# Codeuser0717/CVAE-GAN

Measured on NVIDIA B200. Metric: train_samples_per_s, higher is better.
Workload: dtype f32

## Files before the change

cvae_gan_b200/csrc/chain.cuh:

```cuda
#pragma once
#include "gemm.cuh"
#include "misc_kernels.cuh"

namespace cvg {

constexpr int CH_TM = 32;
constexpr int CH_THREADS = 256;
constexpr int CH_NB = 64;
constexpr int CH_KC = 64;
constexpr int CH_H0 = 256, CH_H1 = 128, CH_H2 = 64;
constexpr int CH_MAX_IN = 256;
constexpr int CH_MAX_K = 32;
constexpr int CH_WBUF = 2 * CH_KC * CH_NB;

struct CriticChainArgs {
  int M = 0, ld = 0, F = 0;
  const float* x = nullptr;
  long long sx = 0;
  const float* W[4] = {};
  int ldw[4] = {};
  const float* b[4] = {};
  const float* wlabel = nullptr;
  int ldwl = 0;
  const float* inv_sigma = nullptr;
  const uint8_t* m1 = nullptr;
  const uint8_t* m2 = nullptr;
  float keep_inv = 1.f, slope = 0.2f;
  float* a[3] = {};
  float* s = nullptr;
  float* g[3] = {};
  double* osum = nullptr;
  float seed[2] = {0.f, 0.f};
};

struct ClassifierChainArgs {
  int M = 0, ld = 0, F = 0, K = 0, label = 0;
  const float* x = nullptr;
  long long sx = 0;
  const float* W[4] = {};
  const float* b[4] = {};
  const float* gamma = nullptr;
  const float* beta = nullptr;
  float ln_eps = 1e-5f;
  const uint8_t* m1 = nullptr;
  const uint8_t* m2 = nullptr;
  float keep_inv = 1.f;
  float *a1 = nullptr, *h2 = nullptr, *a2 = nullptr, *rs = nullptr, *a3 = nullptr, *logit = nullptr, *dlogit = nullptr;
  float* g[3] = {};
  float coef = 1.f;
  double* loss = nullptr;
  float* dgamma = nullptr;
  float* dbeta = nullptr;
  unsigned long long* acc = nullptr;
  unsigned* cnt = nullptr;
};

template <bool WT, class Ep>
__device__ __forceinline__ void chain_layer(const float* X, const float* __restrict__ W, int ldw, int R, int N, float* wbuf,
                                            Ep ep) {
  const int tid = threadIdx.x;
  const int grp = tid >> 6, t64 = tid & 63;
  const int tm = (t64 & 7) * 4, tn = (t64 >> 3) * 8;
  const int Rp = (R + TBK - 1) / TBK * TBK;
  const int nkc = (Rp + CH_KC - 1) / CH_KC;
  const bool wvec = (ldw & 3) == 0;
  for (int n0 = 0; n0 < N; n0 += CH_NB) {
    float4 pre[4];
    auto gload = [&](int kc) {
#pragma unroll
      for (int j = 0; j < 4; ++j) pre[j] = make_float4(0.f, 0.f, 0.f, 0.f);
      if (WT) {
        const int n = n0 + (tid & 63);
        if (n >= N) return;
#pragma unroll
        for (int j = 0; j < 4; ++j) {
          const int k = kc + (tid >> 6) * 16 + 4 * j;
          const float* src = W + (size_t)n * ldw + k;
          if (wvec && k + 3 < R) {
            pre[j] = ld4(src);
          } else {
            if (k < R) pre[j].x = src[0];
            if (k + 1 < R) pre[j].y = src[1];
            if (k + 2 < R) pre[j].z = src[2];
            if (k + 3 < R) pre[j].w = src[3];
          }
        }
      } else {
// ... 114 lines not shown
    return tot;
  }
};

struct DactEp {
  float scale;
  const uint8_t* mask;
  float keep_inv;
  float neg;
  const float* A;
  float* Y;
  float* S;
  int ld, m0, M;
  __device__ __forceinline__ void operator()(int n, int m, float4 v) const {
    float y[4] = {v.x, v.y, v.z, v.w};
    const size_t off = (size_t)n * ld + m0 + m;
    float keep[4] = {1.f, 1.f, 1.f, 1.f};
    if (mask) {
      const uchar4 mk = *reinterpret_cast<const uchar4*>(mask + off);
      keep[0] = ep_keep(mk.x, keep_inv);
      keep[1] = ep_keep(mk.y, keep_inv);
      keep[2] = ep_keep(mk.z, keep_inv);
      keep[3] = ep_keep(mk.w, keep_inv);
    }
#pragma unroll
    for (int i = 0; i < 4; ++i) y[i] = ep_dact(y[i], scale, keep[i], A[n * CH_TM + m + i], neg);
    st4(Y + off, make_float4(y[0], y[1], y[2], y[3]));
    if (S)
#pragma unroll
      for (int i = 0; i < 4; ++i) S[n * CH_TM + m + i] = m0 + m + i < M ? y[i] : 0.f;
  }
};

__device__ __forceinline__ void chain_stage(float* S, int rows, const float* src, int nvalid, int ld, int m0, int M) {
  for (int i = threadIdx.x; i < rows * CH_TM; i += CH_THREADS) {
    const int k = i / CH_TM, m = i % CH_TM;
    S[i] = (k < nvalid && m0 + m < M) ? src[(size_t)k * ld + m0 + m] : 0.f;
  }
}

__host__ __device__ inline int chain_x_rows(int F, int K) {
  const int fp = (F + TBK - 1) / TBK * TBK;
  const int kp = 2 * ((K + TBK - 1) / TBK * TBK);
  return fp > kp ? fp : kp;
}
inline size_t critic_chain_smem(int F) {
  return sizeof(float) * ((size_t)CH_WBUF + (size_t)(CH_H0 + CH_H1 + CH_H2) * CH_TM + (size_t)chain_x_rows(F, 1) * CH_TM);
}
inline size_t classifier_chain_smem(int F, int K) {
  return sizeof(float) * ((size_t)CH_WBUF + (size_t)(CH_H0 + 2 * CH_H1 + CH_H2) * CH_TM + (size_t)chain_x_rows(F, K) * CH_TM);
}

__global__ void __launch_bounds__(CH_THREADS, 2) critic_chain_kernel(const CriticChainArgs g) {
  extern __shared__ __align__(16) float ch_smem[];
  float* wbuf = ch_smem;
  float* A0 = wbuf + CH_WBUF;
  float* A1 = A0 + CH_H0 * CH_TM;
  float* A2 = A1 + CH_H1 * CH_TM;
  float* X = A2 + CH_H2 * CH_TM;
  const int pass = blockIdx.y, m0 = blockIdx.x * CH_TM;
  const int M = g.M, ld = g.ld;
  const size_t ps0 = (size_t)pass * CH_H0 * ld, ps1 = (size_t)pass * CH_H1 * ld, ps2 = (size_t)pass * CH_H2 * ld;

  chain_stage(X, (g.F + TBK - 1) / TBK * TBK, g.x + (long long)pass * g.sx, g.F, ld, m0, M);
  __syncthreads();
  chain_layer<true>(X, g.W[0], g.ldw[0], g.F, CH_H0, wbuf,
                    FwdEp{g.b[0], g.wlabel, g.ldwl, g.inv_sigma[0 + pass], ACT_LRELU, g.slope, g.m1 + ps0, g.keep_inv,
                          g.a[0] + ps0, A0, ld, m0, M});
  chain_layer<true>(A0, g.W[1], g.ldw[1], CH_H0, CH_H1, wbuf,
                    FwdEp{g.b[1], nullptr, 0, g.inv_sigma[2 + pass], ACT_LRELU, g.slope, g.m2 + ps1, g.keep_inv,
                          g.a[1] + ps1, A1, ld, m0, M});
  chain_layer<true>(A1, g.W[2], g.ldw[2], CH_H1, CH_H2, wbuf,
                    FwdEp{g.b[2], nullptr, 0, g.inv_sigma[4 + pass], ACT_LRELU, g.slope, nullptr, 1.f,
                          g.a[2] + ps2, A2, ld, m0, M});
  double tot = 0.0;
  const FwdEp score{g.b[3], nullptr, 0, g.inv_sigma[6 + pass], ACT_NONE, g.slope, nullptr, 1.f,
                    g.s + (size_t)pass * ld, nullptr, ld, m0, M};
  chain_layer<true>(A2, g.W[3], g.ldw[3], CH_H2, 1, wbuf, [&](int n, int m, float4 y) { tot += score(n, m, y); });
  tot = warp_sum_d(tot);
  if (threadIdx.x == 0) atomicAdd(g.osum + pass, tot);
  for (int i = threadIdx.x; i < TBK * CH_TM; i += CH_THREADS)
    X[i] = (i < CH_TM && m0 + i < M) ? g.seed[pass] : 0.f;
  __syncthreads();
  chain_layer<false>(X, g.W[3], g.ldw[3], 1, CH_H2, wbuf,
                     DactEp{g.inv_sigma[6 + pass], nullptr, 1.f, g.slope, A2, g.g[2] + ps2, A2, ld, m0, M});
  chain_layer<false>(A2, g.W[2], g.ldw[2], CH_H2, CH_H1, wbuf,
                     DactEp{g.inv_sigma[4 + pass], g.m2 + ps1, g.keep_inv, g.slope, A1, g.g[1] + ps1, A1, ld, m0, M});
  chain_layer<false>(A1, g.W[1], g.ldw[1], CH_H1, CH_H0, wbuf,
                     DactEp{g.inv_sigma[2 + pass], g.m1 + ps0, g.keep_inv, g.slope, A0, g.g[0] + ps0, nullptr, ld, m0, M});
}

__global__ void __launch_bounds__(CH_THREADS, 2) classifier_chain_kernel(const ClassifierChainArgs g) {
  extern __shared__ __align__(16) float ch_smem[];
  __shared__ float red1[8][LN_ROWS], red2[8][LN_ROWS];
  __shared__ unsigned s_last;
  float* wbuf = ch_smem;
  float* A1 = wbuf + CH_WBUF;
  float* H2 = A1 + CH_H0 * CH_TM;
  float* A2 = H2 + CH_H1 * CH_TM;
  float* A3 = A2 + CH_H1 * CH_TM;
  float* X = A3 + CH_H2 * CH_TM;
  const int Kp = (g.K + TBK - 1) / TBK * TBK;
  float* L = X;
  float* D = X + Kp * CH_TM;
  const int pass = blockIdx.y, m0 = blockIdx.x * CH_TM;
  const int M = g.M, ld = g.ld;
  const int lane = threadIdx.x & 31, w = threadIdx.x >> 5;
  const bool valid = m0 + lane < M;
  const size_t ps0 = (size_t)pass * CH_H0 * ld, ps1 = (size_t)pass * CH_H1 * ld, ps2 = (size_t)pass * CH_H2 * ld;
  const size_t psk = (size_t)pass * g.K * ld;

  chain_stage(X, (g.F + TBK - 1) / TBK * TBK, g.x + (long long)pass * g.sx, g.F, ld, m0, M);
  for (int i = threadIdx.x; i < CH_H1 * CH_TM; i += CH_THREADS) A2[i] = 0.f;
  __syncthreads();
  chain_layer<true>(X, g.W[0], g.F, g.F, CH_H0, wbuf,
                    FwdEp{g.b[0], nullptr, 0, 1.0f, ACT_RELU, 0.f, g.m1 + ps0, g.keep_inv, g.a1 + ps0, A1, ld, m0, M});
  chain_layer<true>(A1, g.W[1], CH_H0, CH_H0, CH_H1, wbuf,
                    FwdEp{g.b[1], nullptr, 0, 1.0f, ACT_NONE, 0.f, nullptr, 1.f, g.h2 + ps1, H2, ld, m0, M});
  float mean, rstd;
  {
    const uint8_t* mk = g.m2 + ps1 + m0 + lane;
    float* a2g = g.a2 + ps1 + m0 + lane;
    ln_fwd_row<LN_MAXF>(
        CH_H1, valid, g.ln_eps, g.gamma, g.beta, mk, ld, g.keep_inv, red1, [&](int c) { return H2[c * CH_TM + lane]; },
        [&](int c, float n) {
          a2g[(size_t)c * ld] = n;
          A2[c * CH_TM + lane] = n;
        },
        mean, rstd);
    if (valid && w == 0) {
      float* rs = g.rs + (size_t)pass * 2 * ld;
      rs[m0 + lane] = mean;
      rs[ld + m0 + lane] = rstd;
    }
  }
  for (int i = threadIdx.x; i < Kp * CH_TM; i += CH_THREADS) D[i] = 0.f;
  __syncthreads();
  chain_layer<true>(A2, g.W[2], CH_H1, CH_H1, CH_H2, wbuf,
                    FwdEp{g.b[2], nullptr, 0, 1.0f, ACT_RELU, 0.f, nullptr, 1.f, g.a3 + ps2, A3, ld, m0, M});
  chain_layer<true>(A3, g.W[3], CH_H2, CH_H2, g.K, wbuf,
                    FwdEp{g.b[3], nullptr, 0, 1.0f, ACT_NONE, 0.f, nullptr, 1.f, g.logit + psk, L, ld, m0, M});
  if (w == 0) {
    double nll = 0.0;
    if (valid) {
      nll = ce_row(L + lane, CH_TM, D + lane, CH_TM, g.K, g.label, g.coef);
      float* dg = g.dlogit + psk + m0 + lane;
      for (int k = 0; k < g.K; ++k) dg[(size_t)k * ld] = D[k * CH_TM + lane];
    }
    nll = warp_sum_d(nll);
    if (lane == 0 && nll != 0.0) atomicAdd(g.loss + pass, nll);
  }
  __syncthreads();
  chain_layer<false>(D, g.W[3], CH_H2, g.K, CH_H2, wbuf,
                     DactEp{1.0f, nullptr, 1.f, 0.f, A3, g.g[2] + ps2, A3, ld, m0, M});
  chain_layer<false>(A3, g.W[2], CH_H1, CH_H2, CH_H1, wbuf,
                     DactEp{1.0f, g.m2 + ps1, g.keep_inv, 0.f, A2, g.g[1] + ps1, A2, ld, m0, M});
  {
    float* dhg = g.g[1] + ps1 + m0 + lane;
    ln_bwd_row<LN_MAXF>(
        CH_H1, valid, mean, rstd, g.gamma, red1, red2, [&](int c) { return A2[c * CH_TM + lane]; },
        [&](int c) { return H2[c * CH_TM + lane]; },
        [&](int c, float v) {
          dhg[(size_t)c * ld] = v;
          A2[c * CH_TM + lane] = v;
        },
        g.dgamma ? g.acc : nullptr);
  }
  if (g.dgamma) {
    __threadfence();
    __syncthreads();
    if (threadIdx.x == 0) s_last = atomicAdd(g.cnt, 1u) == gridDim.x * gridDim.y - 1 ? 1u : 0u;
    __syncthreads();
    if (s_last) {
      __threadfence();
      for (int e = threadIdx.x; e < 2 * CH_H1; e += CH_THREADS) {
        const float v = det_unfix(__ldcg(g.acc + e));
        g.acc[e] = 0ull;
        atomicAdd(e < CH_H1 ? g.dgamma + e : g.dbeta + (e - CH_H1), v);
      }
      if (threadIdx.x == 0) *g.cnt = 0u;
    }
  }
  __syncthreads();
  chain_layer<false>(A2, g.W[1], CH_H0, CH_H1, CH_H0, wbuf,
                     DactEp{1.0f, g.m1 + ps0, g.keep_inv, 0.f, A1, g.g[0] + ps0, nullptr, ld, m0, M});
}

}
```

cvae_gan_b200/csrc/engine.cuh:

```cuda
#pragma once
#include "common.cuh"
#include "gemm.cuh"
#include "misc_kernels.cuh"
#include "comm_nvl.cuh"

typedef struct ncclComm* ncclComm_t;

namespace cvg {

constexpr int HOIST_MAX = 16;
constexpr int STAT_C = 1024;

constexpr int DET_MAX_PASS = 4;

struct Workspace {
  int ld = 0;
  int rows_cap = 0;
  float* xT = nullptr;
  float* z = nullptr;
  uint8_t* d_m1 = nullptr;
  uint8_t* d_m2 = nullptr;
  uint8_t* c_m1 = nullptr;
  uint8_t* c_m2 = nullptr;
  float *g_h[3] = {nullptr, nullptr, nullptr};
  float* g_out = nullptr;
  float* hz = nullptr;
  float* hh[3] = {nullptr, nullptr, nullptr};
  float* hout = nullptr;
  double* hfst = nullptr;
  float *g_dy[3] = {nullptr, nullptr, nullptr};
  float* g_dout = nullptr;
  float *e_h[3] = {nullptr, nullptr, nullptr};
  float* e_ml = nullptr;
  float *e_dy[3] = {nullptr, nullptr, nullptr};
  float* e_dml = nullptr;
  float *d_a[3] = {nullptr, nullptr, nullptr};
  float* d_s = nullptr;
  float *d_g[3] = {nullptr, nullptr, nullptr};
  float* c_a1 = nullptr;
  float* c_h2 = nullptr;
  float* c_a2 = nullptr;
  float* c_rs = nullptr;
  float* c_a3 = nullptr;
  float* c_logit = nullptr;
  float* c_dlogit = nullptr;
  float *c_g[3] = {nullptr, nullptr, nullptr};
  float* dx = nullptr;
  float* sn_sigma = nullptr;
  float* sn_inv_sigma = nullptr;
  float* sn_u = nullptr;
  float* sn_v = nullptr;
  long long sn_snap = 0;
  float* sn_G = nullptr;
  double* acc = nullptr;
  size_t acc_bytes = 0;
  double* loss = nullptr;
  double* g_fst = nullptr;
  double* g_bst = nullptr;
  double* e_fst = nullptr;
  double* e_bst = nullptr;
  unsigned long long* gen_count = nullptr;
  StepCtl* ctl = nullptr;
  float* x_stage = nullptr;
  float* tc_w = nullptr;
  float* tc_c = nullptr;
  float* dw_scratch = nullptr;
  long long dw_scratch_floats = 0;
  unsigned long long* det_acc[3] = {};
  unsigned* det_cnt[3] = {};
  long long det_acc_n = 0;
  int det_cnt_n = 0;
  unsigned int* mk_bar = nullptr;
  float* z_eps = nullptr;
  float* mk_wprep = nullptr;
  long long mk_wprep_floats = 0;
  long long* mk_dbg = nullptr;
};

struct MkSlot {
  void* dev = nullptr;
// ... 181 lines not shown
```

cvae_gan_b200/csrc/layout.cu:

```cuda
#include "engine.cuh"

namespace cvg {

static thread_local std::string g_err;
void set_error(const std::string& msg) { g_err = msg; }
const char* last_error() { return g_err.c_str(); }

static int64_t pad4(int64_t n) { return (n + 3) & ~(int64_t)3; }

struct Builder {
  NetLayout& L;
  int64_t po = 0, so = 0;
  explicit Builder(NetLayout& l) : L(l) {}
  int64_t add(const std::string& key, int kind, int64_t d0, int64_t d1) {
    CvgTensorDesc t;
    memset(&t, 0, sizeof(t));
    snprintf(t.key, sizeof(t.key), "%s", key.c_str());
    t.kind = kind;
    t.ndim = d1 > 0 ? 2 : 1;
    t.shape[0] = d0;
    t.shape[1] = d1 > 0 ? d1 : 0;
    const int64_t n = d0 * (d1 > 0 ? d1 : 1);
    int64_t& o = kind == 0 ? po : so;
    t.offset = o;
// ... 147 lines not shown
  const int rows = e.cfg.max_batch;
  const size_t ld = (size_t)((rows + 63) / 64) * 64;
  w.ld = (int)ld;
  w.rows_cap = rows;
  const int F = e.F, K = e.K, Z = e.Z;
  w.xT = c.take<float>(F * ld);
  w.z = c.take<float>(2 * Z * ld);
  w.d_m1 = c.take<uint8_t>(2 * e.dh[0] * ld);
  w.d_m2 = c.take<uint8_t>(2 * e.dh[1] * ld);
  w.c_m1 = c.take<uint8_t>(2 * e.ch[0] * ld);
  w.c_m2 = c.take<uint8_t>(2 * e.ch[1] * ld);
  for (int i = 0; i < 3; ++i) {
    w.g_h[i] = c.take<float>(2 * e.gh[i] * ld);
    w.g_dy[i] = c.take<float>(2 * e.gh[i] * ld);
    w.e_h[i] = c.take<float>(e.eh[i] * ld);
    w.e_dy[i] = c.take<float>(e.eh[i] * ld);
    w.d_a[i] = c.take<float>(2 * e.dh[i] * ld);
    w.d_g[i] = c.take<float>(2 * e.dh[i] * ld);
    w.c_g[i] = c.take<float>(2 * e.ch[i] * ld);
  }
  w.g_out = c.take<float>(2 * F * ld);
  w.g_dout = c.take<float>(2 * F * ld);
  w.e_ml = c.take<float>(2 * Z * ld);
  w.e_dml = c.take<float>(2 * Z * ld);
  w.d_s = c.take<float>(2 * ld);
  w.c_a1 = c.take<float>(2 * e.ch[0] * ld);
  w.c_h2 = c.take<float>(2 * e.ch[1] * ld);
  w.c_a2 = c.take<float>(2 * e.ch[1] * ld);
  w.c_rs = c.take<float>(2 * 2 * ld);
  w.c_a3 = c.take<float>(2 * e.ch[2] * ld);
  w.c_logit = c.take<float>(2 * K * ld);
  w.c_dlogit = c.take<float>(2 * K * ld);
  w.dx = c.take<float>(F * ld);
  w.sn_sigma = c.take<float>(8);
  w.sn_inv_sigma = c.take<float>(8);
  long long snap = 0;
  for (int i = 0; i < 4; ++i) {
    const LinearP& p = e.lay[CVG_NET_DISCRIMINATOR].lin[i];
    snap += pad4(p.out > p.in ? p.out : p.in);
  }
  w.sn_snap = snap;
  w.sn_u = c.take<float>(2 * snap);
  w.sn_v = c.take<float>(2 * snap);
  w.sn_G = c.take<float>(2 * e.lay[CVG_NET_DISCRIMINATOR].n_param);
  const size_t n_acc = 16 + (size_t)(3 * 2 + 3 * 2 + 3 + 3) * 2 * STAT_C;
  w.acc = c.take<double>(n_acc);
  w.acc_bytes = n_acc * sizeof(double);
  if (w.acc) {
    w.loss = w.acc;
    w.g_fst = w.acc + 16;
    w.g_bst = w.g_fst + (size_t)3 * 2 * 2 * STAT_C;
    w.e_fst = w.g_bst + (size_t)3 * 2 * 2 * STAT_C;
    w.e_bst = w.e_fst + (size_t)3 * 2 * STAT_C;
  }
  w.gen_count = c.take<unsigned long long>(4);
  w.ctl = c.take<StepCtl>(1);
  w.x_stage = c.take<float>((size_t)rows * F);
  w.tc_w = c.take<float>((size_t)tc_prep_floats(e));
  w.tc_c = c.take<float>((size_t)tc_const_floats());
  {
    long long per = 0;
    for (int net = 0; net < 4; ++net) {
      long long t = 0;
      for (int i = 0; i < e.lay[net].nlin; ++i) {
        const LinearP& p = e.lay[net].lin[i];
        t += (long long)p.out * (((p.in + 15) & ~15) + 1);
// ... 57 lines not shown
```

cvae_gan_b200/csrc/misc_kernels.cuh:

```cuda
#pragma once
#include "common.cuh"

namespace cvg {

struct StepCtl {
  unsigned long long seed;
  unsigned long long counter;
  long long adam_t[4];
  float lambda_class;
  float pad;
};

__global__ void ctl_set_kernel(StepCtl* c, unsigned long long seed, unsigned long long counter, int set_rng,
                               float lambda_class, int set_lambda) {
  if (threadIdx.x == 0) {
    if (set_rng) { c->seed = seed; c->counter = counter; }
    if (set_lambda) c->lambda_class = lambda_class;
  }
}
__global__ void ctl_bump_kernel(StepCtl* c, unsigned long long dcounter, int adam_mask) {
  if (threadIdx.x == 0) {
    c->counter += dcounter;
    for (int n = 0; n < 4; ++n)
      if (adam_mask & (1 << n)) c->adam_t[n] += 1;
// ... 197 lines not shown
};

__device__ __forceinline__ double ce_row(const float* l, size_t ldl, float* d, size_t ldd, int K, int tgt, float coef) {
  float mx = -INFINITY;
  for (int k = 0; k < K; ++k) mx = fmaxf(mx, l[(size_t)k * ldl]);
  float s = 0.f;
  for (int k = 0; k < K; ++k) s += expf(l[(size_t)k * ldl] - mx);
  const float lse = logf(s);
  const double nll = -(double)(l[(size_t)tgt * ldl] - mx - lse);
  for (int k = 0; k < K; ++k) {
    const float p = expf(l[(size_t)k * ldl] - mx - lse);
    d[(size_t)k * ldd] = (p - (k == tgt ? 1.f : 0.f)) * coef;
  }
  return nll;
}

__global__ void ce_kernel(const CeArgs g) {
  const int m = blockIdx.x * blockDim.x + threadIdx.x;
  const int pass = blockIdx.y;
  double nll = 0.0;
  if (m < g.M) {
    const int tgt = g.labels ? (int)g.labels[m] : g.label;
    const float coef = g.ctl ? g.coef * g.ctl->lambda_class : g.coef;
    nll = ce_row(g.logits + (long long)pass * g.sl + m, g.ld, g.dlogits + (long long)pass * g.sd + m, g.ld, g.K, tgt, coef);
  }
  nll = warp_sum_d(nll);
  if ((threadIdx.x & 31) == 0 && nll != 0.0) atomicAdd(g.loss + pass, nll);
}

struct SeedArgs {
  int M, ld, F;
  const float* out; long long sout;
  const float* x;
  const float* dx;
  float* dpre; long long sdpre;
  float coef_recon;
  double* recon_acc;
  int prior_only = 0;
  int add_dx = 0;
};

__global__ void g_seed_kernel(const SeedArgs g) {
  const int idx = blockIdx.x * blockDim.x + threadIdx.x;
  const int pass = blockIdx.y;
  const int f = idx / g.ld, m = idx % g.ld;
  double sq = 0.0;
  if (f < g.F) {
    const size_t off = (size_t)f * g.ld + m;
    float d = 0.f;
    if (m < g.M) {
      const float o = g.out[(long long)pass * g.sout + off];
      float dout;
      if (pass == 0 && !g.prior_only) {
        const float diff = o - g.x[off];
        sq = (double)diff * (double)diff;
        dout = g.coef_recon * 2.0f * diff;
        if (g.add_dx) dout += g.dx[off];
      } else {
        dout = g.dx[off];
      }
      d = dout * (1.0f - o) * o;
    }
    g.dpre[(long long)pass * g.sdpre + off] = d;
  }
  if (pass == 0 && !g.prior_only) {
    sq = warp_sum_d(sq);
    if ((threadIdx.x & 31) == 0 && sq != 0.0) atomicAdd(g.recon_acc, sq);
  }
}

constexpr int SN_MAXDIM = 1024;
struct SnLayer {
  const float* W; int rows, cols;
  float* u; float* v;
  int snap_off;
};
struct SnArgs {
  SnLayer L[4];
  int npass, do_power;
  float eps;
  float* sigma;
  float* inv_sigma;
  float* u_snap; float* v_snap; long long ssnap;
  int w_smem_floats = 0;
};

constexpr int SN_THREADS = 1024;

__global__ void __launch_bounds__(SN_THREADS) sn_power_kernel(const SnArgs g) {
  __shared__ float su[SN_MAXDIM], sv[SN_MAXDIM], st[SN_MAXDIM];
  __shared__ float part[SN_THREADS];
  __shared__ double red[32];
// ... 595 lines not shown
```

cvae_gan_b200/csrc/train.cu:

```cuda
#include <dlfcn.h>
#include <math.h>

#include "chain.cuh"
#include "engine.cuh"
#include "mega.cuh"

namespace cvg {

#define CVG_PAR(e) do { (e).mk.par_next = true; } while (0)

struct Id128 {
  char b[128];
};
struct NcclApi {
  int (*GetUniqueId)(void*) = nullptr;
  int (*CommInitRank)(ncclComm_t*, int, Id128, int) = nullptr;
  int (*AllReduce)(const void*, void*, size_t, int, int, ncclComm_t, cudaStream_t) = nullptr;
  int (*CommDestroy)(ncclComm_t) = nullptr;
  const char* (*GetErrorString)(int) = nullptr;
  bool ok = false;
};
static NcclApi g_nccl;

static int load_nccl() {
// ... 621 lines not shown
    } else {
      g.a.p = w.c_a3; g.a.sp = (long long)p.in * ld;
      g.Y = w.c_logit;
    }
    CVG_TRY(launch_mn(e, true, g, st));
    if (l == 1) {
      LnArgs a;
      a.M = M; a.ld = w.ld; a.C = p.out; a.npass = npass;
      a.h = w.c_h2; a.sh = (long long)p.out * ld;
      a.g = e.P(net, p.gamma); a.b = e.P(net, p.beta);
      a.eps = e.cfg.ln_eps;
      a.mask = train ? w.c_m2 : nullptr; a.smask = (long long)p.out * ld; a.keep_inv = keep_inv;
      a.a = w.c_a2; a.sa = (long long)p.out * ld;
      a.rs = w.c_rs; a.srs = 2 * (long long)ld;
      if (e.mk.recording) {
        CVG_TRY(mk_push(e, mk::K_LN_FWD, &a, sizeof(a), npass * ((M + 31) / 32)));
      } else {
        launch_ln_fwd(a, st);
        CVG_LAUNCH_CHECK();
      }
    }
  }
  return 0;
}

static bool chain_usable(const Engine& e, int net) {
  if (!e.chain || e.mk.recording) return false;
  const int* h = net == CVG_NET_DISCRIMINATOR ? e.dh : e.ch;
  return h[0] == CH_H0 && h[1] == CH_H1 && h[2] == CH_H2 && e.F <= CH_MAX_IN && e.K <= CH_MAX_K;
}

static cudaStream_t chain_dw_stream(Engine& e, int l, cudaStream_t st) { return l == 1 ? st : fork_to(e, l == 2 ? 1 : 0, st); }

static int launch_critic_chain(Engine& e, long long sx, int label, int M, const float* seed, cudaStream_t st) {
  const int net = CVG_NET_DISCRIMINATOR;
  const Workspace& w = e.ws;
  CriticChainArgs a;
  a.M = M; a.ld = w.ld; a.F = e.F;
  a.x = w.xT; a.sx = sx;
  double flops = 0.0;
  for (int l = 0; l < 4; ++l) {
    const LinearP& p = lin(e, net, l);
    a.W[l] = e.P(net, p.w); a.ldw[l] = p.in; a.b[l] = e.P(net, p.b);
    flops += 2.0 * ((l == 0) ? e.F : p.in) * p.out + (l > 0 ? 2.0 * p.in * p.out : 0.0);
  }
  a.wlabel = label_column(e, net, lin(e, net, 0), e.F, label);
  a.ldwl = lin(e, net, 0).in;
  a.inv_sigma = w.sn_inv_sigma;
  a.m1 = w.d_m1; a.m2 = w.d_m2;
  a.keep_inv = 1.0f / (1.0f - e.cfg.dropout_p);
  a.slope = e.cfg.lrelu_slope;
  for (int i = 0; i < 3; ++i) { a.a[i] = w.d_a[i]; a.g[i] = w.d_g[i]; }
  a.s = w.d_s;
  a.osum = w.loss + L_DREAL;
  a.seed[0] = seed[0]; a.seed[1] = seed[1];
  const dim3 grid(2 * ((M + TBM - 1) / TBM), 2);
  prof_begin(e, 3, flops * 2 * M, st);
  critic_chain_kernel<<<grid, CH_THREADS, critic_chain_smem(e.F), st>>>(a);
  prof_end(e, st);
  CVG_LAUNCH_CHECK();
  return 0;
}

static int launch_classifier_chain(Engine& e, long long sx, int label, int M, float coef, cudaStream_t st) {
  const int net = CVG_NET_CLASSIFIER;
  const Workspace& w = e.ws;
  ClassifierChainArgs a;
  a.M = M; a.ld = w.ld; a.F = e.F; a.K = e.K; a.label = label;
  a.x = w.xT; a.sx = sx;
  double flops = 0.0;
  for (int l = 0; l < 4; ++l) {
    const LinearP& p = lin(e, net, l);
    a.W[l] = e.P(net, p.w); a.b[l] = e.P(net, p.b);
    flops += 2.0 * p.in * p.out * (l > 0 ? 2.0 : 1.0);
  }
  const LinearP& p1 = lin(e, net, 1);
  a.gamma = e.P(net, p1.gamma); a.beta = e.P(net, p1.beta);
  a.ln_eps = e.cfg.ln_eps;
  a.m1 = w.c_m1; a.m2 = w.c_m2;
  a.keep_inv = 1.0f / (1.0f - e.cfg.dropout_p);
  a.a1 = w.c_a1; a.h2 = w.c_h2; a.a2 = w.c_a2; a.rs = w.c_rs; a.a3 = w.c_a3; a.logit = w.c_logit; a.dlogit = w.c_dlogit;
  for (int i = 0; i < 3; ++i) a.g[i] = w.c_g[i];
  a.coef = coef;
  a.loss = w.loss + L_CE0;
  a.dgamma = e.G(net, p1.gamma); a.dbeta = e.G(net, p1.beta);
  const int slot = det_slot(e, st);
  if (2LL * CH_H1 > e.ws.det_acc_n) CVG_FAIL("internal: LayerNorm backward exceeds the deterministic-reduction slots");
  a.acc = e.ws.det_acc[slot]; a.cnt = e.ws.det_cnt[slot];
  const dim3 grid(2 * ((M + TBM - 1) / TBM), 2);
  prof_begin(e, 3, flops * 2 * M, st);
  classifier_chain_kernel<<<grid, CH_THREADS, classifier_chain_smem(e.F, e.K), st>>>(a);
  prof_end(e, st);
  CVG_LAUNCH_CHECK();
  return 0;
}

static int bwd_critic(Engine& e, const float* xin, long long sxin, int npass, int label, int M, const float* seed,
                      bool want_dw, bool want_dx, cudaStream_t st, bool dw_only = false) {
  const int net = CVG_NET_DISCRIMINATOR;
  const Workspace& w = e.ws;
  const size_t ld = w.ld;
  const float keep_inv = 1.0f / (1.0f - e.cfg.dropout_p);
  const long long sG = e.lay[net].n_param;
  for (int l = 3; l >= 0; --l) {
    const LinearP& p = lin(e, net, l);
    Operand dy;
    if (l == 3) {
      dy.kind = OP_CONST; dy.rows = 1; dy.cst = seed[0];
    } else {
      dy.kind = OP_PLAIN; dy.rows = p.out; dy.p = w.d_g[l]; dy.sp = (long long)p.out * ld;
    }
    if (want_dw) {
      const int reps = (l == 3 && npass > 1) ? npass : 1;
      const cudaStream_t sw = dw_only ? chain_dw_stream(e, l, st) : fork_to(e, 0, st);
      for (int r = 0; r < reps; ++r) {
        if (r > 0) CVG_PAR(e);
        DwArgs d = base_dw(e, M, (float)M, reps > 1 ? 1 : npass);
        d.N = p.out;
        d.K = (l == 0) ? e.F : p.in;
        d.p = dy;
        if (l == 3) d.p.cst = seed[reps > 1 ? r : 0];
        d.q.kind = OP_PLAIN;
        d.q.rows = d.K;
        if (l == 0) { d.q.p = xin + (reps > 1 ? r * sxin : 0); d.q.sp = sxin; }
// ... 405 lines not shown

int step_d(Engine& e, const float* x_real, int label, int B, const CvgNoise* nz, const StepRng& rng, int flags,
           float* loss_out, cudaStream_t st) {
  CVG_TRY(check_step(e, B));
  ProgramScope prog(e);
  CVG_TRY(begin_step(e, rng, false, st));
  const Workspace& w = e.ws;
  const bool local_bn = flags & CVG_STEP_LOCAL_BN;
  const float Bg = (float)B * (float)e.world;
  const float Bg_bn = local_bn ? (float)B : Bg;
  const int D = CVG_NET_DISCRIMINATOR;
  if (rng.set) CVG_PAR(e);
  CVG_TRY(emit_zero(e, w.acc, w.acc_bytes, st));
  CVG_PAR(e);
  CVG_TRY(emit_zero(e, w.sn_G, sizeof(float) * 2 * e.lay[D].n_param, st));
  CVG_TRY(prep_net(e, CVG_NET_GENERATOR, true, false, false));
  CVG_TRY(prep_net(e, D, true, true, false));
  FillArgs f;
  fill_args(e, f, rng, B);
  if (!e.hoist_x) add_job(f, w.z, nz ? nz->z : nullptr, 0, e.Z, 1, RS_Z);
  add_job(f, w.d_m1, nz ? nz->d_mask1 : nullptr, 1, e.dh[0], 2, RS_DMASK1);
  add_job(f, w.d_m2, nz ? nz->d_mask2 : nullptr, 1, e.dh[1], 2, RS_DMASK2);
  CVG_PAR(e);
  CVG_TRY(launch_fill(e, f, st));
  CVG_PAR(e);
  CVG_TRY(stage_x(e, x_real, B, fork_to(e, 1, st)));
  CVG_PAR(e);
  CVG_TRY(launch_sn(e, 2, true, fork_to(e, 0, st)));
  if (!e.hoist_x) CVG_TRY(fwd_generator(e, 1, true, false, label, B, Bg_bn, local_bn, st));
  join_sides(e, st);
  const long long sx = (e.hoist_x ? e.hoist_x : w.g_out) - w.xT;
  const float seedv[2] = {-1.0f / Bg, 1.0f / Bg};
  if (chain_usable(e, D)) {
    CVG_TRY(launch_critic_chain(e, sx, label, B, seedv, st));
    CVG_TRY(bwd_critic(e, w.xT, sx, 2, label, B, seedv, true, false, st, true));
  } else {
    CVG_TRY(fwd_critic(e, w.xT, sx, 2, label, B, w.loss + L_DREAL, st));
    CVG_TRY(bwd_critic(e, w.xT, sx, 2, label, B, seedv, true, false, st));
  }
  join_sides(e, st);
  {
    SnGradArgs a;
    int off = 0;
    for (int l = 0; l < 4; ++l) {
      const LinearP& p = lin(e, D, l);
      a.L[l].W = e.P(D, p.w); a.L[l].rows = p.out; a.L[l].cols = p.in;
      a.L[l].u = nullptr; a.L[l].v = nullptr; a.L[l].snap_off = off;
      off += ((p.out > p.in ? p.out : p.in) + 3) & ~3;
      a.w_off[l] = p.w;
    }
    a.npass = 2;
    a.Gp = w.sn_G; a.sG = e.lay[D].n_param;
    a.inv_sigma = w.sn_inv_sigma;
    a.u_snap = w.sn_u; a.v_snap = w.sn_v; a.ssnap = w.sn_snap;
    a.grad = e.buf[D].grads;
    a.last_bias_grad = e.G(D, lin(e, D, 3).b);
    a.last_bias_value = (float)B * (seedv[0] + seedv[1]);
    double* dots = w.loss + 8;
    if (e.mk.recording) {
      CVG_TRY(mk_emit_dwred(e));
      CVG_TRY(mk_push(e, mk::K_SN_DOT, &a, sizeof(a), mk::SN_DOT_VB * 4 * 2, 0, 0, 0, 0, &dots, sizeof(dots)));
      CVG_TRY(mk_push(e, mk::K_SN_GRAD, &a, sizeof(a), mk::SN_GRAD_VB * 4, 0, 0, 0, 0, &dots, sizeof(dots)));
      CVG_PAR(e);
    } else {
      sn_dot_kernel<<<dim3(16, 4, 2), 256, 0, st>>>(a, dots);
      CVG_LAUNCH_CHECK();
      sn_grad_kernel<<<dim3(32, 4), 256, 0, st>>>(a, dots);
// ... 2 lines not shown
  }
  CVG_TRY(finish_step(e, 1 << D, 0, B, flags, loss_out, st));
  return prog.finish(st);
}

int step_c(Engine& e, const float* x_real, int label, int B, const CvgNoise* nz, const StepRng& rng, int flags,
           float* loss_out, cudaStream_t st) {
  CVG_TRY(check_step(e, B));
  ProgramScope prog(e);
  CVG_TRY(begin_step(e, rng, false, st));
  const Workspace& w = e.ws;
  const size_t ld = w.ld;
  const bool local_bn = flags & CVG_STEP_LOCAL_BN;
  const float Bg = (float)B * (float)e.world;
  const float Bg_bn = local_bn ? (float)B : Bg;
  const int C = CVG_NET_CLASSIFIER;
  if (rng.set) CVG_PAR(e);
  CVG_TRY(emit_zero(e, w.acc, w.acc_bytes, st));
  CVG_TRY(prep_net(e, CVG_NET_GENERATOR, true, false, false));
  CVG_TRY(prep_net(e, C, true, true, false));
  FillArgs f;
  fill_args(e, f, rng, B);
  if (!e.hoist_x) add_job(f, w.z, nz ? nz->z : nullptr, 0, e.Z, 1, RS_Z);
  add_job(f, w.c_m1, nz ? nz->c_mask1 : nullptr, 1, e.ch[0], 2, RS_CMASK1);
  add_job(f, w.c_m2, nz ? nz->c_mask2 : nullptr, 1, e.ch[1], 2, RS_CMASK2);
  CVG_PAR(e);
  CVG_TRY(launch_fill(e, f, st));
  CVG_PAR(e);
  CVG_TRY(stage_x(e, x_real, B, fork_to(e, 1, st)));
  if (!e.hoist_x) CVG_TRY(fwd_generator(e, 1, true, false, label, B, Bg_bn, local_bn, st));
  join_sides(e, st);
  const long long sx = (e.hoist_x ? e.hoist_x : w.g_out) - w.xT;
  if (chain_usable(e, C)) {
    CVG_TRY(launch_classifier_chain(e, sx, label, B, 1.0f / Bg, st));
    CVG_TRY(bwd_classifier(e, w.xT, sx, 2, B, true, false, false, st, nullptr, true));
  } else {
    CVG_TRY(fwd_classifier(e, w.xT, sx, 2, true, B, st));
    CeArgs c;
    c.M = B; c.ld = w.ld; c.K = e.K; c.npass = 2; c.label = label;
    c.logits = w.c_logit; c.sl = (long long)e.K * ld;
    c.dlogits = w.c_dlogit; c.sd = (long long)e.K * ld;
    c.coef = 1.0f / Bg;
    c.ctl = nullptr;
    c.loss = w.loss + L_CE0;
    CVG_TRY(emit_ce(e, c, B, 2, st));
    CVG_TRY(bwd_classifier(e, w.xT, sx, 2, B, true, false, false, st));
  }
  CVG_TRY(finish_step(e, 1 << C, 1, B, flags, loss_out, st));
  return prog.finish(st);
}

int step_classifier(Engine& e, const float* x, const long long* labels, int B, const CvgNoise* nz, const StepRng& rng,
                    const AdamOverride& ov, int flags, float* loss_out, cudaStream_t st) {
  if (!e.ws_base) CVG_FAIL("workspace not bound");
  if (B < 1 || B > e.ws.rows_cap) CVG_FAIL("batch size exceeds max_batch");
  ProgramScope prog(e);
  CVG_TRY(begin_step(e, rng, false, st));
  const Workspace& w = e.ws;
  const size_t ld = w.ld;
  const int C = CVG_NET_CLASSIFIER;
  const float Bg = (float)B * (float)e.world;
  if (rng.set) CVG_PAR(e);
  CVG_TRY(emit_zero(e, w.acc, w.acc_bytes, st));
  CVG_TRY(prep_net(e, C, true, true, false));
  FillArgs f;
  fill_args(e, f, rng, B);
  add_job(f, w.c_m1, nz ? nz->c_mask1 : nullptr, 1, e.ch[0], 1, RS_CMASK1);
// ... 159 lines not shown
  CVG_TRY(begin_step(e, rng, true, st));
  const Workspace& w = e.ws;
  const size_t ld = w.ld;
  const bool local_bn = flags & CVG_STEP_LOCAL_BN;
  const float Bg = (float)B * (float)e.world;
  const float Bg_bn = local_bn ? (float)B : Bg;
  const int E = CVG_NET_ENCODER, G = CVG_NET_GENERATOR;
  if (rng.set) CVG_PAR(e);
  CVG_TRY(emit_zero(e, w.acc, w.acc_bytes, st));
  CVG_TRY(prep_net(e, E, true, true, false));
  CVG_TRY(prep_net(e, G, true, true, true));
  CVG_TRY(prep_net(e, CVG_NET_DISCRIMINATOR, true, true, true));
  CVG_TRY(prep_net(e, CVG_NET_CLASSIFIER, true, rng.lambda_nonzero, true));
  FillArgs f;
  fill_args(e, f, rng, B);
  add_job(f, e.mk.recording ? w.z_eps : w.z, nz ? nz->eps : nullptr, 0, e.Z, 1, RS_EPS);
  add_job(f, w.z + (size_t)e.Z * ld, nz ? nz->z : nullptr, 0, e.Z, 1, RS_Z);
  add_job(f, w.d_m1, nz ? nz->d_mask1 : nullptr, 1, e.dh[0], 1, RS_DMASK1);
  add_job(f, w.d_m2, nz ? nz->d_mask2 : nullptr, 1, e.dh[1], 1, RS_DMASK2);
  add_job(f, w.c_m1, nz ? nz->c_mask1 : nullptr, 1, e.ch[0], 1, RS_CMASK1);
  add_job(f, w.c_m2, nz ? nz->c_mask2 : nullptr, 1, e.ch[1], 1, RS_CMASK2);
  CVG_PAR(e);
  CVG_TRY(launch_fill(e, f, st));
  const float* x_fake = w.g_out + (size_t)e.F * ld;
  CeArgs c;
  c.M = B; c.ld = w.ld; c.K = e.K; c.npass = 1; c.label = label;
  c.logits = w.c_logit; c.sl = (long long)e.K * ld;
  c.dlogits = w.c_dlogit; c.sd = (long long)e.K * ld;
  c.coef = 1.0f / Bg;
  c.ctl = w.ctl;
  c.loss = w.loss + L_CE0;
  const float seedv[2] = {-e.cfg.lambda_adv / Bg, 0.f};
  const bool three = !e.mk.recording && e.ms.on && (e.world <= 1 || local_bn || fold_stats(e, local_bn));
  join_sides(e, st);
  if (three) {
    const cudaStream_t sA = fork_to(e, 0, st), sB = fork_to(e, 1, st);
    CVG_TRY(launch_sn(e, 1, true, sA));
    CVG_TRY(stage_x(e, x_real, B, sB));
    wait_for(e, st, sB);
    GenSplit prior;
    prior.only_pass = 1; prior.channel = 1; prior.rec = e.ms.layer;
    CVG_TRY(fwd_generator(e, 2, true, false, label, B, Bg_bn, local_bn, sB, nullptr, &prior));
    wait_for(e, sB, sA);
    if (rng.lambda_nonzero) {
      wait_for(e, sA, sB);
      CVG_TRY(fwd_classifier(e, x_fake, 0, 1, true, B, sA));
      CVG_TRY(emit_ce(e, c, B, 1, sA));
    }
    CVG_TRY(fwd_critic(e, x_fake, 0, 1, label, B, w.loss + L_DFAKE, sB));
    CVG_TRY(bwd_critic(e, x_fake, 0, 1, label, B, seedv, false, true, sB));
    if (rng.lambda_nonzero) CVG_TRY(bwd_classifier(e, x_fake, 0, 1, B, false, true, true, sA, sB));
    CVG_TRY(fwd_encoder(e, true, label, B, Bg_bn, local_bn, st));
    GenSplit enc;
    enc.only_pass = 0; enc.channel = 0; enc.wait = e.ms.layer;
    CVG_TRY(fwd_generator(e, 2, true, true, label, B, Bg_bn, local_bn, st, nullptr, &enc));
    join_sides(e, st);
  } else {
  CVG_PAR(e);
  CVG_TRY(stage_x(e, x_real, B, fork_to(e, 1, st)));

  CVG_PAR(e);
  CVG_TRY(launch_sn(e, 1, true, fork_to(e, 0, st)));
  join_sides(e, st, 1);
  CVG_TRY(fwd_encoder(e, true, label, B, Bg_bn, local_bn, st));
  if (e.mk.recording) {
    mk::ReparamArgs ra;
    ra.mu = w.e_ml; ra.lv = w.e_ml + (size_t)e.Z * ld; ra.eps = w.z_eps; ra.out = w.z; ra.M = B; ra.ld = w.ld; ra.Z = e.Z;
    CVG_TRY(mk_push(e, mk::K_REPARAM, &ra, sizeof(ra), (int)(((long long)e.Z * ld + mk::THREADS - 1) / mk::THREADS)));
  }
  CVG_TRY(fwd_generator(e, 2, true, true, label, B, Bg_bn, local_bn, st));
  join_sides(e, st);
  const cudaStream_t sc = rng.lambda_nonzero ? fork_to(e, 1, st) : st;
  CVG_TRY(fwd_critic(e, x_fake, 0, 1, label, B, w.loss + L_DFAKE, st));
  CVG_TRY(fwd_classifier(e, x_fake, 0, 1, true, B, sc));
  CVG_TRY(emit_ce(e, c, B, 1, sc));
  CVG_TRY(bwd_critic(e, x_fake, 0, 1, label, B, seedv, false, true, st));
  if (rng.lambda_nonzero) CVG_TRY(bwd_classifier(e, x_fake, 0, 1, B, false, true, true, sc, st));
  join_sides(e, st);
  }

  SeedArgs s;
  s.M = B; s.ld = w.ld; s.F = e.F;
  s.out = w.g_out; s.sout = (long long)e.F * ld;
  s.x = w.xT; s.dx = w.dx;
  s.dpre = w.g_dout; s.sdpre = (long long)e.F * ld;
  s.coef_recon = e.cfg.lambda_recon / (Bg * (float)e.F);
  s.recon_acc = w.loss + L_RECON;
  if (e.mk.recording) {
    CVG_TRY(mk_push(e, mk::K_SEED, &s, sizeof(s), 2 * (int)(((long long)e.F * ld + mk::THREADS - 1) / mk::THREADS)));
  } else {
    g_seed_kernel<<<dim3((unsigned)((e.F * ld + 255) / 256), 2), 256, 0, st>>>(s);
    CVG_LAUNCH_CHECK();
  }

  const LinearP& g0 = lin(e, G, 0);
  BnNetBwd gb;
  gb.net = G; gb.npass = 2;
  gb.h = w.g_h; gb.dy = w.g_dy;
  gb.top_dy = w.g_dout; gb.s_top = (long long)e.F * ld;
  gb.first_in.kind = e.mk.recording ? OP_PLAIN : OP_REPARAM; gb.first_in.rows = e.Z;
  gb.first_in.p = w.z; gb.first_in.sp = (long long)e.Z * ld;
  gb.first_in.mu = w.e_ml; gb.first_in.lv = w.e_ml + (size_t)e.Z * ld; gb.first_in.eps = w.z;
  gb.first_in.reparam_pass = 0;
  gb.first_K = e.Z;
  gb.label_col = label_col_index(e, e.Z, label);
  gb.want_first_dx = true;
  (void)g0;
  CVG_TRY(bwd_bn_net(e, gb, B, Bg_bn, e.cfg.lambda_kl / Bg, local_bn, st));

  BnNetBwd eb;
  eb.net = E; eb.npass = 1;
  eb.h = w.e_h; eb.dy = w.e_dy;
  eb.top_dy = w.e_dml; eb.s_top = 0;
  eb.first_in.kind = OP_PLAIN; eb.first_in.rows = e.F; eb.first_in.p = w.xT;
  eb.first_K = e.F;
  eb.label_col = label_col_index(e, e.F, label);
  eb.want_first_dx = false;
  CVG_TRY(bwd_bn_net(e, eb, B, Bg_bn, 0.f, local_bn, st));

  CVG_TRY(finish_step(e, (1 << E) | (1 << G), 2, B, flags, loss_out, st));
// ... 46 lines not shown
      } else if (e.mk.recording) {
        e.mk.src_rows = class_rows; e.mk.src_n = n_rows; e.mk.src_Bg = B_global; e.mk.src_off = (long long)e.rank * B;
        x = class_rows;
      } else {
        sample_rows_kernel<<<(B + 127) / 128, 128, 0, fork_to(e, 1, st)>>>(class_rows, n_rows, B_global, (long long)e.rank * B,
                                                                            B, e.F, 0, 0, e.ws.ctl, 0, e.ws.x_stage, nullptr);
        CVG_LAUNCH_CHECK();
        x = e.ws.x_stage;
      }
      StepRng rng;
      rng.set = false;
      rng.off = 1;
      rng.lambda_nonzero = !(flags & CVG_VISIT_LAMBDA_ZERO);
      float* lo = loss_out ? loss_out + 4 * i : nullptr;
      const int sf = flags & (CVG_STEP_LOCAL_BN | CVG_STEP_NO_UPDATE | CVG_STEP_PRIOR_ONLY | CVG_STEP_CVAE);
      if (!e.mk.recording) e.step_dcounter = 2;
      if (kind == 0) CVG_TRY(step_d(e, x, label, B, nullptr, rng, sf, lo, st));
      else if (kind == 1) CVG_TRY(step_c(e, x, label, B, nullptr, rng, sf, lo, st));
      else CVG_TRY(step_g(e, x, label, B, nullptr, rng, sf, lo, st));
      e.mk.src_rows = nullptr;
      e.hoist_x = nullptr;
      if (e.mk.recording) {
        e.mk.dcounter += 2;
      }
    }
  }
  join_sides(e, st);
  return prog.finish(st);
}

void set_all_kernel_attributes() {
  mk_set_kernel_attributes();
  cudaFuncSetAttribute(sn_power_kernel, cudaFuncAttributeMaxDynamicSharedMemorySize, SN_W_SMEM_MAX);
  cudaFuncSetAttribute(critic_chain_kernel, cudaFuncAttributeMaxDynamicSharedMemorySize, (int)critic_chain_smem(CH_MAX_IN));
  cudaFuncSetAttribute(classifier_chain_kernel, cudaFuncAttributeMaxDynamicSharedMemorySize,
                       (int)classifier_chain_smem(CH_MAX_IN, CH_MAX_K));
#define CVG_MN_ATTR(W, A, E) cudaFuncSetAttribute(gemm_mn_kernel<W, A, E>, cudaFuncAttributeMaxDynamicSharedMemorySize, 112 * 1024);
  CVG_MN_ATTR(true, OP_PLAIN, EP_LINEAR) CVG_MN_ATTR(true, OP_BN_ACT, EP_LINEAR) CVG_MN_ATTR(true, OP_REPARAM, EP_LINEAR)
  CVG_MN_ATTR(false, OP_PLAIN, EP_DACT) CVG_MN_ATTR(false, OP_CONST, EP_DACT) CVG_MN_ATTR(false, OP_PLAIN, EP_STORE)
  CVG_MN_ATTR(false, OP_PLAIN, EP_DBN) CVG_MN_ATTR(false, OP_BN_BWD, EP_DBN) CVG_MN_ATTR(false, OP_BN_BWD, EP_REPARAM_BWD)
#undef CVG_MN_ATTR
#define CVG_DW_ATTR(P, Q) cudaFuncSetAttribute(gemm_dw_kernel<P, Q>, cudaFuncAttributeMaxDynamicSharedMemorySize, 100 * 1024);
  CVG_DW_ATTR(OP_PLAIN, OP_PLAIN) CVG_DW_ATTR(OP_CONST, OP_PLAIN) CVG_DW_ATTR(OP_PLAIN, OP_BN_ACT)
  CVG_DW_ATTR(OP_BN_BWD, OP_BN_ACT) CVG_DW_ATTR(OP_BN_BWD, OP_REPARAM) CVG_DW_ATTR(OP_BN_BWD, OP_PLAIN)
#undef CVG_DW_ATTR
}

}
```

Measured before the change: 12.88 million.

## Use fused critic/classifier chain kernels for generator step with input-gradient output

Templates the critic and classifier chain kernels on an input-gradient mode, which adds a final layer-0 backward that writes dx for fake samples. The generator step's separate forward/backward critic and classifier launches are replaced with single chain launches on parallel streams. The classifier's dx goes to a new buffer that the seed kernel adds into dx. This cuts kernel launches and global round-trips of activations, but each chain block now recomputes an extra GEMM with limited parallelism.

```diff
diff --git a/cvae_gan_b200/csrc/chain.cuh b/cvae_gan_b200/csrc/chain.cuh
--- a/cvae_gan_b200/csrc/chain.cuh
+++ b/cvae_gan_b200/csrc/chain.cuh
@@ -31,6 +31,7 @@
   float* g[3] = {};
   double* osum = nullptr;
   float seed[2] = {0.f, 0.f};
+  float* dx = nullptr;
 };
 
 struct ClassifierChainArgs {
@@ -53,6 +54,8 @@
   float* dbeta = nullptr;
   unsigned long long* acc = nullptr;
   unsigned* cnt = nullptr;
+  const StepCtl* ctl = nullptr;
+  float* dx = nullptr;
 };
 
 template <bool WT, class Ep>
@@ -233,6 +236,15 @@
   }
 };
 
+struct StoreEp {
+  float scale;
+  float* Y;
+  int ld, m0;
+  __device__ __forceinline__ void operator()(int n, int m, float4 v) const {
+    st4(Y + (size_t)n * ld + m0 + m, make_float4(v.x * scale, v.y * scale, v.z * scale, v.w * scale));
+  }
+};
+
 __device__ __forceinline__ void chain_stage(float* S, int rows, const float* src, int nvalid, int ld, int m0, int M) {
   for (int i = threadIdx.x; i < rows * CH_TM; i += CH_THREADS) {
     const int k = i / CH_TM, m = i % CH_TM;
@@ -252,6 +264,7 @@
   return sizeof(float) * ((size_t)CH_WBUF + (size_t)(CH_H0 + 2 * CH_H1 + CH_H2) * CH_TM + (size_t)chain_x_rows(F, K) * CH_TM);
 }
 
+template <bool EG>
 __global__ void __launch_bounds__(CH_THREADS, 2) critic_chain_kernel(const CriticChainArgs g) {
   extern __shared__ __align__(16) float ch_smem[];
   float* wbuf = ch_smem;
@@ -288,9 +301,13 @@
   chain_layer<false>(A2, g.W[2], g.ldw[2], CH_H2, CH_H1, wbuf,
                      DactEp{g.inv_sigma[4 + pass], g.m2 + ps1, g.keep_inv, g.slope, A1, g.g[1] + ps1, A1, ld, m0, M});
   chain_layer<false>(A1, g.W[1], g.ldw[1], CH_H1, CH_H0, wbuf,
-                     DactEp{g.inv_sigma[2 + pass], g.m1 + ps0, g.keep_inv, g.slope, A0, g.g[0] + ps0, nullptr, ld, m0, M});
-}
-
+                     DactEp{g.inv_sigma[2 + pass], g.m1 + ps0, g.keep_inv, g.slope, A0, g.g[0] + ps0, EG ? A0 : nullptr,
+                            ld, m0, M});
+  if (EG)
+    chain_layer<false>(A0, g.W[0], g.ldw[0], CH_H0, g.F, wbuf, StoreEp{g.inv_sigma[0 + pass], g.dx, ld, m0});
+}
+
+template <bool EG>
 __global__ void __launch_bounds__(CH_THREADS, 2) classifier_chain_kernel(const ClassifierChainArgs g) {
   extern __shared__ __align__(16) float ch_smem[];
   __shared__ float red1[8][LN_ROWS], red2[8][LN_ROWS];
@@ -344,7 +361,7 @@
   if (w == 0) {
     double nll = 0.0;
     if (valid) {
-      nll = ce_row(L + lane, CH_TM, D + lane, CH_TM, g.K, g.label, g.coef);
+      nll = ce_row(L + lane, CH_TM, D + lane, CH_TM, g.K, g.label, EG ? g.coef * g.ctl->lambda_class : g.coef);
       float* dg = g.dlogit + psk + m0 + lane;
       for (int k = 0; k < g.K; ++k) dg[(size_t)k * ld] = D[k * CH_TM + lane];
     }
@@ -384,7 +401,8 @@
   }
   __syncthreads();
   chain_layer<false>(A2, g.W[1], CH_H0, CH_H1, CH_H0, wbuf,
-                     DactEp{1.0f, g.m1 + ps0, g.keep_inv, 0.f, A1, g.g[0] + ps0, nullptr, ld, m0, M});
-}
-
-}
+                     DactEp{1.0f, g.m1 + ps0, g.keep_inv, 0.f, A1, g.g[0] + ps0, EG ? A1 : nullptr, ld, m0, M});
+  if (EG) chain_layer<false>(A1, g.W[0], g.F, CH_H0, g.F, wbuf, StoreEp{1.0f, g.dx, ld, m0});
+}
+
+}
diff --git a/cvae_gan_b200/csrc/engine.cuh b/cvae_gan_b200/csrc/engine.cuh
--- a/cvae_gan_b200/csrc/engine.cuh
+++ b/cvae_gan_b200/csrc/engine.cuh
@@ -46,6 +46,7 @@
   float* c_dlogit = nullptr;
   float *c_g[3] = {nullptr, nullptr, nullptr};
   float* dx = nullptr;
+  float* dx_c = nullptr;
   float* sn_sigma = nullptr;
   float* sn_inv_sigma = nullptr;
   float* sn_u = nullptr;
diff --git a/cvae_gan_b200/csrc/layout.cu b/cvae_gan_b200/csrc/layout.cu
--- a/cvae_gan_b200/csrc/layout.cu
+++ b/cvae_gan_b200/csrc/layout.cu
@@ -203,6 +203,7 @@
   w.c_logit = c.take<float>(2 * K * ld);
   w.c_dlogit = c.take<float>(2 * K * ld);
   w.dx = c.take<float>(F * ld);
+  w.dx_c = c.take<float>(F * ld);
   w.sn_sigma = c.take<float>(8);
   w.sn_inv_sigma = c.take<float>(8);
   long long snap = 0;
diff --git a/cvae_gan_b200/csrc/misc_kernels.cuh b/cvae_gan_b200/csrc/misc_kernels.cuh
--- a/cvae_gan_b200/csrc/misc_kernels.cuh
+++ b/cvae_gan_b200/csrc/misc_kernels.cuh
@@ -253,12 +253,13 @@
   int M, ld, F;
   const float* out; long long sout;
   const float* x;
-  const float* dx;
+  float* dx;
   float* dpre; long long sdpre;
   float coef_recon;
   double* recon_acc;
   int prior_only = 0;
   int add_dx = 0;
+  const float* dx_c = nullptr;
 };
 
 __global__ void g_seed_kernel(const SeedArgs g) {
@@ -279,6 +280,10 @@
         if (g.add_dx) dout += g.dx[off];
       } else {
         dout = g.dx[off];
+        if (g.dx_c) {
+          dout += g.dx_c[off];
+          g.dx[off] = dout;
+        }
       }
       d = dout * (1.0f - o) * o;
     }
diff --git a/cvae_gan_b200/csrc/train.cu b/cvae_gan_b200/csrc/train.cu
--- a/cvae_gan_b200/csrc/train.cu
+++ b/cvae_gan_b200/csrc/train.cu
@@ -677,17 +677,18 @@
 
 static cudaStream_t chain_dw_stream(Engine& e, int l, cudaStream_t st) { return l == 1 ? st : fork_to(e, l == 2 ? 1 : 0, st); }
 
-static int launch_critic_chain(Engine& e, long long sx, int label, int M, const float* seed, cudaStream_t st) {
+static int launch_critic_chain(Engine& e, const float* x, long long sx, int npass, int label, int M, const float* seed,
+                               double* osum, bool eg, cudaStream_t st) {
   const int net = CVG_NET_DISCRIMINATOR;
   const Workspace& w = e.ws;
   CriticChainArgs a;
   a.M = M; a.ld = w.ld; a.F = e.F;
-  a.x = w.xT; a.sx = sx;
+  a.x = x; a.sx = sx;
   double flops = 0.0;
   for (int l = 0; l < 4; ++l) {
     const LinearP& p = lin(e, net, l);
     a.W[l] = e.P(net, p.w); a.ldw[l] = p.in; a.b[l] = e.P(net, p.b);
-    flops += 2.0 * ((l == 0) ? e.F : p.in) * p.out + (l > 0 ? 2.0 * p.in * p.out : 0.0);
+    flops += 2.0 * ((l == 0) ? e.F : p.in) * p.out * ((l > 0 || eg) ? 2.0 : 1.0);
   }
   a.wlabel = label_column(e, net, lin(e, net, 0), e.F, label);
   a.ldwl = lin(e, net, 0).in;
@@ -697,27 +698,33 @@
   a.slope = e.cfg.lrelu_slope;
   for (int i = 0; i < 3; ++i) { a.a[i] = w.d_a[i]; a.g[i] = w.d_g[i]; }
   a.s = w.d_s;
-  a.osum = w.loss + L_DREAL;
+  a.osum = osum;
   a.seed[0] = seed[0]; a.seed[1] = seed[1];
-  const dim3 grid(2 * ((M + TBM - 1) / TBM), 2);
-  prof_begin(e, 3, flops * 2 * M, st);
-  critic_chain_kernel<<<grid, CH_THREADS, critic_chain_smem(e.F), st>>>(a);
+  const dim3 grid(2 * ((M + TBM - 1) / TBM), npass);
+  prof_begin(e, 3, flops * npass * M, st);
+  if (eg) {
+    a.dx = w.dx;
+    critic_chain_kernel<true><<<grid, CH_THREADS, critic_chain_smem(e.F), st>>>(a);
+  } else {
+    critic_chain_kernel<false><<<grid, CH_THREADS, critic_chain_smem(e.F), st>>>(a);
+  }
   prof_end(e, st);
   CVG_LAUNCH_CHECK();
   return 0;
 }
 
-static int launch_classifier_chain(Engine& e, long long sx, int label, int M, float coef, cudaStream_t st) {
+static int launch_classifier_chain(Engine& e, const float* x, long long sx, int npass, int label, int M, float coef, bool eg,
+                                   cudaStream_t st) {
   const int net = CVG_NET_CLASSIFIER;
   const Workspace& w = e.ws;
   ClassifierChainArgs a;
   a.M = M; a.ld = w.ld; a.F = e.F; a.K = e.K; a.label = label;
-  a.x = w.xT; a.sx = sx;
+  a.x = x; a.sx = sx;
   double flops = 0.0;
   for (int l = 0; l < 4; ++l) {
     const LinearP& p = lin(e, net, l);
     a.W[l] = e.P(net, p.w); a.b[l] = e.P(net, p.b);
-    flops += 2.0 * p.in * p.out * (l > 0 ? 2.0 : 1.0);
+    flops += 2.0 * p.in * p.out * ((l > 0 || eg) ? 2.0 : 1.0);
   }
   const LinearP& p1 = lin(e, net, 1);
   a.gamma = e.P(net, p1.gamma); a.beta = e.P(net, p1.beta);
@@ -728,13 +735,19 @@
   for (int i = 0; i < 3; ++i) a.g[i] = w.c_g[i];
   a.coef = coef;
   a.loss = w.loss + L_CE0;
-  a.dgamma = e.G(net, p1.gamma); a.dbeta = e.G(net, p1.beta);
-  const int slot = det_slot(e, st);
-  if (2LL * CH_H1 > e.ws.det_acc_n) CVG_FAIL("internal: LayerNorm backward exceeds the deterministic-reduction slots");
-  a.acc = e.ws.det_acc[slot]; a.cnt = e.ws.det_cnt[slot];
-  const dim3 grid(2 * ((M + TBM - 1) / TBM), 2);
-  prof_begin(e, 3, flops * 2 * M, st);
-  classifier_chain_kernel<<<grid, CH_THREADS, classifier_chain_smem(e.F, e.K), st>>>(a);
+  const dim3 grid(2 * ((M + TBM - 1) / TBM), npass);
+  prof_begin(e, 3, flops * npass * M, st);
+  if (eg) {
+    a.ctl = w.ctl;
+    a.dx = w.dx_c;
+    classifier_chain_kernel<true><<<grid, CH_THREADS, classifier_chain_smem(e.F, e.K), st>>>(a);
+  } else {
+    a.dgamma = e.G(net, p1.gamma); a.dbeta = e.G(net, p1.beta);
+    const int slot = det_slot(e, st);
+    if (2LL * CH_H1 > e.ws.det_acc_n) CVG_FAIL("internal: LayerNorm backward exceeds the deterministic-reduction slots");
+    a.acc = e.ws.det_acc[slot]; a.cnt = e.ws.det_cnt[slot];
+    classifier_chain_kernel<false><<<grid, CH_THREADS, classifier_chain_smem(e.F, e.K), st>>>(a);
+  }
   prof_end(e, st);
   CVG_LAUNCH_CHECK();
   return 0;
@@ -1206,7 +1219,7 @@
   const long long sx = (e.hoist_x ? e.hoist_x : w.g_out) - w.xT;
   const float seedv[2] = {-1.0f / Bg, 1.0f / Bg};
   if (chain_usable(e, D)) {
-    CVG_TRY(launch_critic_chain(e, sx, label, B, seedv, st));
+    CVG_TRY(launch_critic_chain(e, w.xT, sx, 2, label, B, seedv, w.loss + L_DREAL, false, st));
     CVG_TRY(bwd_critic(e, w.xT, sx, 2, label, B, seedv, true, false, st, true));
   } else {
     CVG_TRY(fwd_critic(e, w.xT, sx, 2, label, B, w.loss + L_DREAL, st));
@@ -1275,7 +1288,7 @@
   join_sides(e, st);
   const long long sx = (e.hoist_x ? e.hoist_x : w.g_out) - w.xT;
   if (chain_usable(e, C)) {
-    CVG_TRY(launch_classifier_chain(e, sx, label, B, 1.0f / Bg, st));
+    CVG_TRY(launch_classifier_chain(e, w.xT, sx, 2, label, B, 1.0f / Bg, false, st));
     CVG_TRY(bwd_classifier(e, w.xT, sx, 2, B, true, false, false, st, nullptr, true));
   } else {
     CVG_TRY(fwd_classifier(e, w.xT, sx, 2, true, B, st));
@@ -1501,6 +1514,7 @@
   c.loss = w.loss + L_CE0;
   const float seedv[2] = {-e.cfg.lambda_adv / Bg, 0.f};
   const bool three = !e.mk.recording && e.ms.on && (e.world <= 1 || local_bn || fold_stats(e, local_bn));
+  const bool c_chain = three && rng.lambda_nonzero && chain_usable(e, CVG_NET_CLASSIFIER);
   join_sides(e, st);
   if (three) {
     const cudaStream_t sA = fork_to(e, 0, st), sB = fork_to(e, 1, st);
@@ -1513,12 +1527,20 @@
     wait_for(e, sB, sA);
     if (rng.lambda_nonzero) {
       wait_for(e, sA, sB);
-      CVG_TRY(fwd_classifier(e, x_fake, 0, 1, true, B, sA));
-      CVG_TRY(emit_ce(e, c, B, 1, sA));
-    }
-    CVG_TRY(fwd_critic(e, x_fake, 0, 1, label, B, w.loss + L_DFAKE, sB));
-    CVG_TRY(bwd_critic(e, x_fake, 0, 1, label, B, seedv, false, true, sB));
-    if (rng.lambda_nonzero) CVG_TRY(bwd_classifier(e, x_fake, 0, 1, B, false, true, true, sA, sB));
+      if (c_chain) {
+        CVG_TRY(launch_classifier_chain(e, x_fake, 0, 1, label, B, c.coef, true, sA));
+      } else {
+        CVG_TRY(fwd_classifier(e, x_fake, 0, 1, true, B, sA));
+        CVG_TRY(emit_ce(e, c, B, 1, sA));
+      }
+    }
+    if (chain_usable(e, CVG_NET_DISCRIMINATOR)) {
+      CVG_TRY(launch_critic_chain(e, x_fake, 0, 1, label, B, seedv, w.loss + L_DFAKE, true, sB));
+    } else {
+      CVG_TRY(fwd_critic(e, x_fake, 0, 1, label, B, w.loss + L_DFAKE, sB));
+      CVG_TRY(bwd_critic(e, x_fake, 0, 1, label, B, seedv, false, true, sB));
+    }
+    if (rng.lambda_nonzero && !c_chain) CVG_TRY(bwd_classifier(e, x_fake, 0, 1, B, false, true, true, sA, sB));
     CVG_TRY(fwd_encoder(e, true, label, B, Bg_bn, local_bn, st));
     GenSplit enc;
     enc.only_pass = 0; enc.channel = 0; enc.wait = e.ms.layer;
@@ -1555,6 +1577,7 @@
   s.dpre = w.g_dout; s.sdpre = (long long)e.F * ld;
   s.coef_recon = e.cfg.lambda_recon / (Bg * (float)e.F);
   s.recon_acc = w.loss + L_RECON;
+  s.dx_c = c_chain ? w.dx_c : nullptr;
   if (e.mk.recording) {
     CVG_TRY(mk_push(e, mk::K_SEED, &s, sizeof(s), 2 * (int)(((long long)e.F * ld + mk::THREADS - 1) / mk::THREADS)));
   } else {
@@ -1667,8 +1690,11 @@
 void set_all_kernel_attributes() {
   mk_set_kernel_attributes();
   cudaFuncSetAttribute(sn_power_kernel, cudaFuncAttributeMaxDynamicSharedMemorySize, SN_W_SMEM_MAX);
-  cudaFuncSetAttribute(critic_chain_kernel, cudaFuncAttributeMaxDynamicSharedMemorySize, (int)critic_chain_smem(CH_MAX_IN));
-  cudaFuncSetAttribute(classifier_chain_kernel, cudaFuncAttributeMaxDynamicSharedMemorySize,
+  cudaFuncSetAttribute(critic_chain_kernel<false>, cudaFuncAttributeMaxDynamicSharedMemorySize, (int)critic_chain_smem(CH_MAX_IN));
+  cudaFuncSetAttribute(critic_chain_kernel<true>, cudaFuncAttributeMaxDynamicSharedMemorySize, (int)critic_chain_smem(CH_MAX_IN));
+  cudaFuncSetAttribute(classifier_chain_kernel<false>, cudaFuncAttributeMaxDynamicSharedMemorySize,
+                       (int)classifier_chain_smem(CH_MAX_IN, CH_MAX_K));
+  cudaFuncSetAttribute(classifier_chain_kernel<true>, cudaFuncAttributeMaxDynamicSharedMemorySize,
                        (int)classifier_chain_smem(CH_MAX_IN, CH_MAX_K));
 #define CVG_MN_ATTR(W, A, E) cudaFuncSetAttribute(gemm_mn_kernel<W, A, E>, cudaFuncAttributeMaxDynamicSharedMemorySize, 112 * 1024);
   CVG_MN_ATTR(true, OP_PLAIN, EP_LINEAR) CVG_MN_ATTR(true, OP_BN_ACT, EP_LINEAR) CVG_MN_ATTR(true, OP_REPARAM, EP_LINEAR)
```

Result: no change. 12.98 million, median of 6 (+0.7%).
